# ftl/sdrainer

Measured on AMD Instinct MI355X. Metric: IQ MSamples/s through FFT+peak+envelope, higher is better.
Workload: dtype f64

## Files before the change

sdrainer_amd/csrc/bank.h:

```cpp
#pragma once
#include <hip/hip_runtime.h>

#include <algorithm>
#include <atomic>
#include <chrono>
#include <cmath>
#include <cstdio>
#include <cstdlib>
#include <cstring>
#include <memory>
#include <mutex>
#include <string>
#include <thread>
#include <vector>

#include "../../include/sdrainer_hip.h"
#include "host/delivery.h"
#include "host/frequency_mapping.h"
#include "sdr_device.h"

namespace sdrcapi {

inline thread_local std::string g_last_error;

inline int fail(int code, const std::string &msg)
{
    g_last_error = msg;
    return code;
}
#define HIP_TRY(expr)                                                                                  \
    do {                                                                                               \
        hipError_t _e = (expr);                                                                        \
        if (_e != hipSuccess)                                                                          \
            return fail(SDR_ERR_HIP, std::string(#expr) + ": " + hipGetErrorString(_e));               \
    } while (0)

template <class T>
struct DevBuf {
    T *p = nullptr;
    size_t n = 0;
    hipError_t alloc(size_t count)
    {
        n = count;
        if (count == 0)
            return hipSuccess;
        hipError_t e = hipMalloc(reinterpret_cast<void **>(&p), count * sizeof(T));
        if (e != hipSuccess)
            return e;
        e = hipMemset(p, 0, count * sizeof(T));
        if (e != hipSuccess)
            return e;
        return hipStreamSynchronize(nullptr);
    }
    void release()
    {
        if (p)
            (void)hipFree(p);
        p = nullptr;
    }
};

inline int ilog2(int n)
{
    int s = 0;
    while ((1 << s) < n)
        s++;
    return s;
}

inline const char *const kKernelNames[sdr::K_COUNT] = {"k_fft_psd",       "k_window_means", "k_noise_stats", "k_thresholds",
                                          "k_listen_gather", "k_cumulate",     "k_find_peaks",  "k_listen_decode"};

constexpr int G_THRESHOLDS = 4, N_GRAPHS = 5;
constexpr int GRAPH_PHASES = 4;
constexpr int RING = 6;
enum Stage { S_FFT = 0, S_NOISE, S_LISTEN, S_PEAKS, N_STAGES };

struct BatchSet {
    DevBuf<float> psd;
    DevBuf<float> tap;
    DevBuf<float> tapw;
    DevBuf<int32_t> tap_used;
    DevBuf<double> win_mean;
    DevBuf<sdr_frame_rec> recs;
    DevBuf<uint64_t> raw_bits, bits;
    DevBuf<sdr_edge> edges;
    DevBuf<uint32_t> edge_counts;
    DevBuf<float> tr_values;
    DevBuf<uint8_t> tr_raw, tr_deb;
    DevBuf<sdr::ListenerSlot> slots_before;
    DevBuf<float> cum_out;
    DevBuf<float> cum_part;
    DevBuf<sdr::DevPeak> dev_peaks;
    DevBuf<int> peak_counts;
    hipEvent_t done[sdr::K_COUNT] = {};
    void release()
    {
        psd.release();
        tap.release();
        tapw.release();
        tap_used.release();
        win_mean.release();
        cum_part.release();
        recs.release();
        raw_bits.release();
        bits.release();
        edges.release();
        edge_counts.release();
        tr_values.release();
        tr_raw.release();
        tr_deb.release();
        slots_before.release();
        cum_out.release();
        dev_peaks.release();
        peak_counts.release();
        for (auto &e : done) {
            if (e)
                (void)hipEventDestroy(e);
            e = nullptr;
        }
    }
};


enum Parts { PART_SPECTRA = 1, PART_LISTEN = 2, PART_ALL = 3 };

struct CursorPack {
    sdr::BatchCursor c[RING];
};

}

struct sdr_bank {
    template <class T>
    using DevBuf = sdrcapi::DevBuf<T>;
    using BatchSet = sdrcapi::BatchSet;
    static constexpr int N_STAGES = sdrcapi::N_STAGES, GRAPH_PHASES = sdrcapi::GRAPH_PHASES, N_GRAPHS = sdrcapi::N_GRAPHS, RING = sdrcapi::RING;

    sdr_config cfg{};
    int logn = 0;
    int device = 0;
    hipStream_t stream[N_STAGES] = {};
    bool own_stream[N_STAGES] = {};

    int max_chunks = 0;
    int text_cap = 2048;
    int edge_cap = 0;
    int bit_words = 0;

    DevBuf<fft64::cplx> tw;
    DevBuf<unsigned char> db_tab;
    DevBuf<int32_t> tap_bins;
    DevBuf<float> spectrum_row;
    std::vector<BatchSet> set;
    DevBuf<sdr::BandState> band_state;
    DevBuf<sdr::ListenerSlot> slots;
    DevBuf<uint16_t> morse;
    DevBuf<uint32_t> text;
    DevBuf<uint32_t> text_frames;
    DevBuf<uint32_t> edge_pos;
    DevBuf<float> carry[2];

    std::vector<sdr::BandState> h_band_state;
    std::vector<sdr::ListenerSlot> h_slots;
    std::vector<int> n_slots;
    std::vector<int64_t> center_frequency;
    int carry_cur = 0;
    int cum_count = 0;
    int64_t total_frames = 0;
    int64_t batch_index = 0;
    int last_set = 0, last_frames = 0, last_chunks = 0, last_count0 = 0;
    int last_carry_in = 0;
    int edge_width = 0;
    int find_peaks = 1;
    bool failed = false;
    DevBuf<sdr::DropCounters> drops;
    DevBuf<sdr::BatchCursor> cursors;
    hipGraph_t graph[GRAPH_PHASES][N_GRAPHS] = {};
    hipGraphExec_t graph_exec[GRAPH_PHASES][N_GRAPHS] = {};
    hipGraphNode_t graph_cursor_node[GRAPH_PHASES] = {};
    hipEvent_t phase_done[GRAPH_PHASES][N_GRAPHS] = {};
    int64_t graph_base = 0;
    int64_t graph_replays = 0;
    bool graph_ready = false;
// ... 95 lines not shown
```

sdrainer_amd/csrc/capi_bank.hip:

```cpp
#include "bank.h"
#include "twiddles.h"

using namespace sdrcapi;

namespace sdr {
int set_error(int code, const char *msg) { return fail(code, msg); }
}

namespace sdrcapi {
std::unique_ptr<host::DeliveryBackend> make_results_backend(sdr_bank *b);

void resolve_profile(sdr_bank *b)
{
    for (auto &p : b->pending) {
        float ms = 0.f;
        if (hipEventElapsedTime(&ms, p.second.first, p.second.second) == hipSuccess) {
            b->prof_ms[p.first] += ms;
            b->prof_n[p.first] += 1;
        }
        (void)hipEventDestroy(p.second.first);
        (void)hipEventDestroy(p.second.second);
    }
    b->pending.clear();
}

int sync_bank(sdr_bank *b)
{
    HIP_TRY(hipSetDevice(b->device));
    {
        const int frc = flush_late_attached(b);
        if (frc)
            return frc;
    }
    for (int s = 0; s < N_STAGES; s++)
        HIP_TRY(hipStreamSynchronize(b->stream[s]));
    resolve_profile(b);
    return SDR_OK;
}

int check_band(sdr_bank *b, int band)
{
    if (!b)
        return fail(SDR_ERR_BAD_ARG, "null bank");
    if (band < 0 || band >= b->cfg.n_bands)
        return fail(SDR_ERR_BAD_ARG, "band out of range");
    return SDR_OK;
}

int check_listener(sdr_bank *b, int band, int lid)
{
    int rc = check_band(b, band);
    if (rc)
        return rc;
    if (lid < 0 || lid >= b->n_slots[band])
        return fail(SDR_ERR_BAD_ARG, "listener id out of range");
    return SDR_OK;
}


hipError_t alloc_set(sdr_bank *b, BatchSet &S)
{
    const sdr_config &c = b->cfg;
    const size_t B = (size_t)c.n_bands, F = (size_t)c.max_batch_frames, L = (size_t)c.max_listeners, N = (size_t)c.block_size;
    hipError_t e = hipSuccess;
#define SET_ALLOC(buf, count)            \
    do {                                 \
        if (e == hipSuccess)             \
            e = (buf).alloc(count);      \
    } while (0)
    SET_ALLOC(S.psd, B * F * N);
    SET_ALLOC(S.tap, B * F * std::max<size_t>(L, 1));
    if (b->logn == 14) {
        SET_ALLOC(S.tapw, B * F * 4 * std::max<size_t>(L, 1));
        SET_ALLOC(S.tap_used, B * std::max<size_t>(L, 1));
    }
    SET_ALLOC(S.win_mean, B * F * 10);
    SET_ALLOC(S.recs, B * F);
    SET_ALLOC(S.raw_bits, B * L * (size_t)b->bit_words);
    SET_ALLOC(S.bits, B * L * (size_t)b->bit_words);
    SET_ALLOC(S.edges, B * L * (size_t)b->edge_cap);
    SET_ALLOC(S.edge_counts, B * L);
    if (c.trace) {
        SET_ALLOC(S.tr_values, B * F * L);
        SET_ALLOC(S.tr_raw, B * F * L);
        SET_ALLOC(S.tr_deb, B * F * L);
        SET_ALLOC(S.slots_before, B * L);
    }
    SET_ALLOC(S.cum_out, B * (size_t)b->max_chunks * N);
    SET_ALLOC(S.cum_part, B * (size_t)b->max_chunks * N);
    SET_ALLOC(S.dev_peaks, B * (size_t)b->max_chunks * (size_t)c.max_peaks);
    SET_ALLOC(S.peak_counts, B * (size_t)b->max_chunks);
#undef SET_ALLOC
#ifndef SDR_STAGE_EVENT_FLAGS
#define SDR_STAGE_EVENT_FLAGS hipEventDisableTiming
#endif
    for (auto &ev : S.done)
        if (e == hipSuccess)
            e = hipEventCreateWithFlags(&ev, SDR_STAGE_EVENT_FLAGS);
    return e;
}

}

extern "C" {
#pragma GCC visibility push(default)

const char *sdr_last_error(void) { return g_last_error.c_str(); }
int sdr_abi_version(void) { return SDR_ABI_VERSION; }
const char *sdr_kernel_name(int kernel) { return (kernel >= 0 && kernel < sdr::K_COUNT) ? kKernelNames[kernel] : ""; }

int sdr_self_check(int device_id)
{
    int ndev = 0;
    HIP_TRY(hipGetDeviceCount(&ndev));
    if (device_id < 0 || device_id >= ndev)
        return fail(SDR_ERR_BAD_ARG, "device_id out of range");
    int prev_dev = 0;
    HIP_TRY(hipGetDevice(&prev_dev));
    struct Restore {
        int dev;
        ~Restore() { (void)hipSetDevice(dev); }
    } restore{prev_dev};
    HIP_TRY(hipSetDevice(device_id));
    unsigned *d = nullptr, h = 0;
    HIP_TRY(hipMalloc(reinterpret_cast<void **>(&d), sizeof(unsigned)));
    hipError_t e = hipMemset(d, 0, sizeof(unsigned));
    const char *ord = getenv("SDR_SELF_CHECK_ORDER");
    if (e == hipSuccess)
        e = sdr::launch_mfma_order_probe(d, ord ? atoi(ord) : 0, nullptr);
    if (e == hipSuccess)
        e = hipMemcpy(&h, d, sizeof h, hipMemcpyDeviceToHost);
    (void)hipFree(d);
    HIP_TRY(e);
    if (h != 0)
        return fail(SDR_ERR_HIP, "self-check failed: v_mfma_f64_4x4x4 does not add its terms as a sequential, individually rounded chain on this "
                                 "device (" + std::to_string(h) + " of 4096 partial sums differ from the vector ALU's); the variance of "
                                 "FindNoiseFloor would not be bit-exact - this part is not supported");
    return SDR_OK;
}

namespace {
static int self_check_once(int device_id)
{
    constexpr int kMax = 64;
    static std::mutex mu;
    static int verdict[kMax];
    static bool done[kMax];
    static std::string message[kMax];
    if (device_id < 0 || device_id >= kMax)
        return sdr_self_check(device_id);
    std::lock_guard<std::mutex> g(mu);
    if (!done[device_id]) {
        verdict[device_id] = sdr_self_check(device_id);
        message[device_id] = g_last_error;
        done[device_id] = verdict[device_id] == SDR_OK || message[device_id].find("self-check failed") != std::string::npos;
    }
    if (verdict[device_id] != SDR_OK)
// ... 441 lines not shown
```

sdrainer_amd/csrc/capi_process.hip:

```cpp
#include <string>

#include "bank.h"

using namespace sdrcapi;

namespace sdrcapi {

constexpr int PUT_SLOTS = 16, PUT_BINS = 128;
struct SlotPack {
    int32_t n;
    int32_t index[PUT_SLOTS];
    sdr::ListenerSlot slot[PUT_SLOTS];
};
struct BinPack {
    int32_t n;
    int32_t index[PUT_BINS], bin[PUT_BINS];
};
__global__ void k_put_slots(sdr::ListenerSlot *slots, SlotPack p)
{
    constexpr int W = sizeof(sdr::ListenerSlot) / 4;
    static_assert(sizeof(sdr::ListenerSlot) % 4 == 0, "word copy");
    for (int i = threadIdx.x; i < p.n * W; i += blockDim.x)
        reinterpret_cast<uint32_t *>(slots + p.index[i / W])[i % W] = reinterpret_cast<const uint32_t *>(&p.slot[i / W])[i % W];
}
// ... 90 lines not shown
        for (int k = 0; k < sdr::K_COUNT && e[k] >= '0' && e[k] < '0' + N_STAGES; k++)
            plan[k] = e[k] - '0';
#define SDR_LAUNCH(id, call) \
    do {                     \
        if (!(diag_skip >> (id) & 1) && SDR_ON(id)) \
            HIP_TRY(call);   \
    } while (0)
#else
#define SDR_LAUNCH(id, call)  \
    do {                      \
        if (SDR_ON(id))       \
            HIP_TRY(call);    \
    } while (0)
#endif
    auto stream_of = [&](int k) { return b->stream[plan[k]]; };
    auto after = [&](int k, int dep) -> int {
        if (stream_of(k) != stream_of(dep) && !cap)
            HIP_TRY(hipStreamWaitEvent(stream_of(k), S.done[dep], 0));
        return SDR_OK;
    };
#define SDR_AFTER(k, dep)          \
    do {                           \
        int _rc = after((k), (dep)); \
        if (_rc)                   \
            return _rc;            \
    } while (0)
    static const bool stop_events = !(getenv("SDR_STOP_EVENTS") && atoi(getenv("SDR_STOP_EVENTS")) == 0);
    const bool ride = stop_events && !cap;
#define SDR_ARM(k) (sdr::t_done_event = ride ? S.done[k] : nullptr)
#define SDR_DONE(k)                                                                                   \
    do {                                                                                              \
        if ((!ride || sdr::t_done_event) && !cap) {                                                   \
            sdr::t_done_event = nullptr;                                                              \
            HIP_TRY(hipEventRecord(S.done[k], stream_of(k)));                                         \
        }                                                                                             \
    } while (0)

    static const bool host_waits = getenv("SDR_HOST_THROTTLE") && atoi(getenv("SDR_HOST_THROTTLE")) != 0;
    int max_slots = 0;
    for (int i = 0; i < B; i++)
        max_slots = std::max(max_slots, b->n_slots[i]);
    if (do_spectra) {
    static const bool park_first = !(getenv("SDR_PARK_FIRST") && atoi(getenv("SDR_PARK_FIRST")) == 0);
    if (b->results_on && !cap && park_first) {
        const int prc = b->results->park(si);
        if (prc)
            return prc;
    }
    {
        static const int launch_order[] = {sdr::K_WINDOW_MEANS, sdr::K_NOISE_STATS, sdr::K_THRESHOLDS, sdr::K_LISTEN_GATHER,
                                           sdr::K_LISTEN_DECODE, sdr::K_CUMULATE,   sdr::K_FIND_PEAKS};
        int last_on[N_STAGES];
        for (int &l : last_on)
            l = -1;
        for (int k : launch_order)
            last_on[plan[k]] = k;
        for (int st = 0; st < N_STAGES; st++) {
            const int k = last_on[st];
            if (k < 0 || st == plan[sdr::K_FFT])
                continue;
            if (cap)
                continue;
            if (hipEventQuery(S.done[k]) == hipSuccess)
                continue;
            if (host_waits)
                HIP_TRY(hipEventSynchronize(S.done[k]));
            else
                HIP_TRY(hipStreamWaitEvent(stream_of(sdr::K_FFT), S.done[k], 0));
        }
    }
    if (b->results_on && !cap && !park_first) {
        const int prc = b->results->park(si);
        if (prc)
            return prc;
    }
    if (cap && SDR_ON(sdr::K_FFT) && capture_k % RING == 0)
        HIP_TRY(launch_set_cursors(b->cursors.p + capture_k, CursorPack{}, stream_of(sdr::K_FFT)));
    {
        ProfScope ps(b, sdr::K_FFT, stream_of(sdr::K_FFT));
        SDR_ARM(sdr::K_FFT);
        sdr::FftTap tap{b->tap_bins.p, S.tap.p, max_slots, c.max_listeners};
        tap.wide = S.tapw.p;
        tap.used = S.tap_used.p;
        SDR_LAUNCH(sdr::K_FFT, sdr::launch_fft(b->logn, iq_dev, cur, b->tw.p, S.psd.p, n_frames, B, in_stride, stride, tap,
                                               stream_of(sdr::K_FFT)));
    }
    SDR_DONE(sdr::K_FFT);

    static const bool scan_path = !(getenv("SDR_NOISE_PATH") && std::string(getenv("SDR_NOISE_PATH")) == "chains");
    static const int force_exact = getenv("SDR_NOISE_FORCE_EXACT") ? atoi(getenv("SDR_NOISE_FORCE_EXACT")) : 0;
    const int scan_count0 = b->cum_count;
    int scan_slots = 1;
    if (n_frames >= SDR_CUMULATION_SIZE - scan_count0)
        scan_slots = 1 + (n_frames - (SDR_CUMULATION_SIZE - scan_count0) + SDR_CUMULATION_SIZE - 1) / SDR_CUMULATION_SIZE;
    if (cap)
        scan_slots = sdr::chunks_completed(SDR_CUMULATION_SIZE - 1, n_frames) + 1;
    const bool scan_bound = scan_path && sdr::cum_bound_pays(n_frames, B, N);
    SDR_AFTER(sdr::K_WINDOW_MEANS, sdr::K_FFT);
    {
        ProfScope ps(b, sdr::K_WINDOW_MEANS, stream_of(sdr::K_WINDOW_MEANS));
        SDR_ARM(sdr::K_WINDOW_MEANS);
        if (scan_path) {
            const sdr::CumGeom scg{N, stride, n_frames, scan_count0, b->max_chunks};
            SDR_LAUNCH(sdr::K_WINDOW_MEANS, sdr::launch_psd_scan(S.psd.p, S.recs.p, S.cum_out.p, S.cum_part.p, cur, ng, scg, scan_slots, B, scan_bound,
                                                                 force_exact, stream_of(sdr::K_WINDOW_MEANS)));
        } else {
            SDR_LAUNCH(sdr::K_WINDOW_MEANS, sdr::launch_window_means(S.psd.p, S.win_mean.p, ng, n_frames, B, stride,
                                                                     stream_of(sdr::K_WINDOW_MEANS)));
        }
    }
    SDR_DONE(sdr::K_WINDOW_MEANS);
    SDR_AFTER(sdr::K_NOISE_STATS, sdr::K_WINDOW_MEANS);
    {
        ProfScope ps(b, sdr::K_NOISE_STATS, stream_of(sdr::K_NOISE_STATS));
        SDR_ARM(sdr::K_NOISE_STATS);
        if (!scan_path)
            SDR_LAUNCH(sdr::K_NOISE_STATS, sdr::launch_noise_stats(S.psd.p, S.win_mean.p, S.recs.p, ng, n_frames, B, stride,
                                                                   stream_of(sdr::K_NOISE_STATS)));
    }
    SDR_DONE(sdr::K_NOISE_STATS);
    SDR_AFTER(sdr::K_THRESHOLDS, sdr::K_NOISE_STATS);
    {
        ProfScope ps(b, sdr::K_THRESHOLDS, stream_of(sdr::K_THRESHOLDS));
        SDR_ARM(sdr::K_THRESHOLDS);
        SDR_LAUNCH(sdr::K_THRESHOLDS, sdr::launch_thresholds(S.recs.p, b->band_state.p, n_frames, B, stride,
                                                             stream_of(sdr::K_THRESHOLDS)));
    }
    SDR_DONE(sdr::K_THRESHOLDS);
    }

    sdr::ListenGeom lg;
    lg.n = N;
    lg.stride = stride;
    lg.max_listeners = c.max_listeners;
    lg.text_cap = b->text_cap;
    lg.edge_cap = b->edge_cap;
    lg.bit_words = b->bit_words;
    lg.trace = c.trace;
    lg.frame_base = (uint32_t)first_frame;
    if (do_listen) {
    SDR_AFTER(sdr::K_LISTEN_GATHER, sdr::K_THRESHOLDS);
    SDR_AFTER(sdr::K_LISTEN_GATHER, sdr::K_FFT);
    SDR_ARM(sdr::K_LISTEN_GATHER);
    if (max_slots > 0) {
        ProfScope ps(b, sdr::K_LISTEN_GATHER, stream_of(sdr::K_LISTEN_GATHER));
        SDR_LAUNCH(sdr::K_LISTEN_GATHER, sdr::launch_listen_gather(S.tap.p, S.psd.p, S.recs.p, b->slots.p, b->db_tab.p, S.raw_bits.p, S.tr_values.p,
                                                                   S.tr_raw.p, cur, lg, n_frames, max_slots, B,
                                                                   stream_of(sdr::K_LISTEN_GATHER)));
    }
    SDR_DONE(sdr::K_LISTEN_GATHER);
    SDR_AFTER(sdr::K_LISTEN_DECODE, sdr::K_LISTEN_GATHER);
    if (c.trace && max_slots > 0 && SDR_ON(sdr::K_LISTEN_DECODE))
        HIP_TRY(hipMemcpyAsync(S.slots_before.p, b->slots.p, sizeof(sdr::ListenerSlot) * (size_t)B * (size_t)c.max_listeners,
                               hipMemcpyDeviceToDevice, stream_of(sdr::K_LISTEN_DECODE)));
    if (!b->results_on)
        SDR_ARM(sdr::K_LISTEN_DECODE);
    if (max_slots > 0) {
        ProfScope ps(b, sdr::K_LISTEN_DECODE, stream_of(sdr::K_LISTEN_DECODE));
        SDR_LAUNCH(sdr::K_LISTEN_DECODE, sdr::launch_listen_decode(b->slots.p, b->morse.p, S.raw_bits.p, S.bits.p, b->text.p,
                                                                   b->text_frames.p, S.edges.p, S.edge_counts.p, S.tr_deb.p, b->drops.p, cur,
                                                                   lg, n_frames, B, b->edge_pos.p, c.max_batch_frames, stream_of(sdr::K_LISTEN_DECODE)));
    }
    if (b->results_on && SDR_ON(sdr::K_LISTEN_DECODE)) {
        SDR_ARM(sdr::K_LISTEN_DECODE);
        HIP_TRY(sdr::launch_pack_listen(b->slots.p, S.edges.p, S.edge_counts.p, b->text.p, b->text_frames.p, b->drops.p, b->res_layout, max_slots, B,
                                        RS.block, stream_of(sdr::K_LISTEN_DECODE)));
// ... 341 lines not shown
```

sdrainer_amd/csrc/k_fft_r32.hip:

```cpp
#include <hip/hip_runtime.h>

#include <algorithm>
#include <cstdlib>
#include <mutex>

#include "fft_r32.h"
#include "sdr_device.h"

#if !defined(SDR_R32_IN_AUX)
#define SDR_R32_IN_AUX 0
#endif
#if !defined(SDR_R32_CHUNK0)
#define SDR_R32_CHUNK0 4
#endif
#if !defined(SDR_R32_PF_PLAN)
#define SDR_R32_PF_PLAN {0, 2, 2, 2, 2, 2, 2, 2, 2, 2, 2, 2, 2, 2, 2, 2, 2}
#endif
#if !defined(SDR_R32_PRIO)
#define SDR_R32_PRIO 1
#endif
#if !defined(SDR_R32_DEPTH2)
#define SDR_R32_DEPTH2 1
#endif
#if !defined(SDR_R32_CHUNK1)
#define SDR_R32_CHUNK1 2
#endif
#if !defined(SDR_R32_PRIO_FLIP2)
#define SDR_R32_PRIO_FLIP2 0
#endif
#if !defined(SDR_R32_PRIO_FLIP1)
#define SDR_R32_PRIO_FLIP1 1
#endif
#if !defined(SDR_R32_CHUNK2)
#define SDR_R32_CHUNK2 4
#endif

namespace sdr {
namespace r32 {

using fft32::cplx;
using rsrc_t = __amdgpu_buffer_rsrc_t;
typedef unsigned u32x2 __attribute__((ext_vector_type(2)));
typedef unsigned u32x4 __attribute__((ext_vector_type(4)));

__device__ __forceinline__ rsrc_t make_rsrc(const void *base, unsigned bytes)
{
    const unsigned long long b = (unsigned long long)base;
    const unsigned lo = __builtin_amdgcn_readfirstlane((unsigned)b), hi = __builtin_amdgcn_readfirstlane((unsigned)(b >> 32));
    return __builtin_amdgcn_make_buffer_rsrc((void *)(((unsigned long long)hi << 32) | lo), 0,
                                             __builtin_amdgcn_readfirstlane(bytes), 0x00020000);
}

__device__ __forceinline__ void wave_sync()
{
    __builtin_amdgcn_fence(__ATOMIC_RELEASE, "wavefront");
    __builtin_amdgcn_wave_barrier();
    __builtin_amdgcn_fence(__ATOMIC_ACQUIRE, "wavefront");
}

enum R32Stamp { RS_TOP = 0, RS_LANDED, RS_CVT, RS_FLUSHED, RS_WIDENED, RS_PASS0, RS_E0, RS_PASS1, RS_E1, RS_PASS2, RS_ROW, RS_STORED, RS_COUNT };
#if defined(SDR_R32_PHASES)
struct R32Stamps {
    unsigned v;
    bool on;
};
#define SDR_R32_STAMP(st, k)                                                                                \
    do {                                                                                                    \
        {                                                                                                   \
            const unsigned now_ = (unsigned)__builtin_amdgcn_s_memtime();                                   \
            asm volatile("v_writelane_b32 %0, %1, %2" : "+v"((st).v) : "s"(now_), "n"((int)(k)));         \
        }                                                                                                   \
    } while (0)
#else
struct R32Stamps {
};
#define SDR_R32_STAMP(st, k) \
    do {                     \
    } while (0)
#endif

constexpr int kPfPoints = 17;
constexpr int kPfPlan[kPfPoints] = SDR_R32_PF_PLAN;
constexpr int pf_begin(int point)
{
    int b = 0;
    for (int i = 0; i < point; i++)
        b += kPfPlan[i];
    return b;
}
static_assert(pf_begin(kPfPoints) == fft32::R, "the prefetch plan must cover the frame's 32 slots");
constexpr int kStorePoints = 7;
#if !defined(SDR_R32_ST_PLAN)
#define SDR_R32_ST_PLAN {2, 1, 1, 1, 1, 1, 1}
#endif
constexpr int kStPlan[kStorePoints] = SDR_R32_ST_PLAN;
constexpr int st_begin(int point)
{
    int b = 0;
    for (int i = 0; i < point; i++)
        b += kStPlan[i];
    return b;
}
static_assert(st_begin(kStorePoints) == fft32::N / 4 / fft32::T, "the store plan must cover the row's eight runs per thread");
enum PfPoint { PF_WIDENED = 0, PF_PASS0 = 1 , PF_E0 = 6 , PF_PRE1 = 10, PF_PASS1 = 11 , PF_POST2 = 15, PF_ROW = 16 };

constexpr int kTw1LdsBytes = fft32::kTw1Entries * 16;
constexpr int kSoftCounters = 4;
constexpr int kLdsBytes = fft32::kExchangeBytes + kTw1LdsBytes + kSoftCounters * 4;
enum SoftId { SOFT_ROW = 0, SOFT_E0 = 1, SOFT_E1 = 2 };
__device__ __forceinline__ void soft_arrive(unsigned *cnt)
{
    unsigned long long save;
    asm volatile("s_waitcnt lgkmcnt(0)\n\t"
                 "s_mov_b64 %0, exec\n\t"
                 "s_mov_b64 exec, 1\n\t"
                 "ds_add_u32 %1, %2\n\t"
                 "s_mov_b64 exec, %0"
                 : "=&s"(save)
                 : "v"((unsigned)(unsigned long long)cnt), "v"(1u)
                 : "memory");
}
__device__ __forceinline__ void soft_wait(unsigned *cnt, unsigned target)
{
    unsigned seen;
    asm volatile("1:\n\t"
                 "ds_read_b32 %0, %1\n\t"
                 "s_waitcnt lgkmcnt(0)\n\t"
                 "v_cmp_lt_u32_e32 vcc, %0, %2\n\t"
                 "s_cbranch_vccz 2f\n\t"
                 "s_sleep 1\n\t"
                 "s_branch 1b\n\t"
                 "2:"
                 : "=&v"(seen)
                 : "v"((unsigned)(unsigned long long)cnt), "v"(target)
                 : "vcc", "memory");
}

__device__ __forceinline__ void set_prio(int stage)
{
#if SDR_R32_PRIO
    unsigned keep;
    if (stage & 1)
        asm volatile("s_cselect_b32 %0, 1, 0\n\ts_cmp_lg_u32 m0, 0\n\ts_cbranch_scc1 1f\n\ts_setprio 1\n\ts_branch 2f\n\t1:\n\ts_setprio 0\n\t2:\n\t"
                     "s_cmp_lg_u32 %0, 0"
                     : "=&s"(keep));
    else
        asm volatile("s_cselect_b32 %0, 1, 0\n\ts_cmp_eq_u32 m0, 0\n\ts_cbranch_scc1 1f\n\ts_setprio 1\n\ts_branch 2f\n\t1:\n\ts_setprio 0\n\t2:\n\t"
                     "s_cmp_lg_u32 %0, 0"
                     : "=&s"(keep));
#endif
}

template <int E, int P>
__device__ __forceinline__ void ex_write(const double (&x)[32], int t, double *area)
{
    const int base = fft32::map_addr_thread<E, P>(t);
#pragma unroll
    for (int s = 0; s < 32; s++)
        area[base + fft32::map_addr_slot<E>(P, s)] = x[s];
}
template <int E, int P>
__device__ __forceinline__ void ex_read(double (&x)[32], int t, const double *area)
{
    const int base = fft32::map_addr_thread<E, P>(t);
#pragma unroll
    for (int s = 0; s < 32; s++)
        x[s] = area[base + fft32::map_addr_slot<E>(P, s)];
}

__global__ __launch_bounds__(fft32::T, 2) void k_fft_r32(const float *__restrict__ iq_arg, const BatchCursor *__restrict__ cur,
                                                          const cplx *__restrict__ tw, float *__restrict__ psd, int in_stride,
                                                          int out_stride, int n_frames, int fpw, const int *__restrict__ tap_bins,
                                                          float *__restrict__ tap_out, int n_tap, int tap_stride,
                                                          float *__restrict__ tap_wide, int *__restrict__ tap_used)
{
#if defined(__HIP_DEVICE_COMPILE__)
    using namespace fft32;
    extern __shared__ __attribute__((aligned(16))) unsigned char smem[];
    double *ex = reinterpret_cast<double *>(smem);
    const unsigned char *tw1_lds = smem + kExchangeBytes;
    const float *__restrict__ iq = cur ? cur->iq : iq_arg;
    const int frame0 = blockIdx.x * fpw;
    const int frame_end = min(frame0 + fpw, n_frames);
    const size_t in_band = (size_t)blockIdx.y * in_stride, out_band = (size_t)blockIdx.y * out_stride;
    const int tid = threadIdx.x;
    const rsrc_t twr = make_rsrc(tw, (unsigned)(kTwTotal * sizeof(cplx)));

    u32x2 pf[R];
    auto fetch = [&](int frame, int t, int m0, int m1) {
        const rsrc_t xrs = make_rsrc(iq + (in_band + frame) * (size_t)N * 2, frame < frame_end ? N * 8u : 0u);
        const unsigned voff = (unsigned)thread_sample(t) * 8u;
#pragma unroll
        for (int m = 0; m < R; m++)
            if (m >= m0 && m < m1)
                pf[m] = __builtin_amdgcn_raw_buffer_load_b64(xrs, voff, slot_sample(m) * 8, SDR_R32_IN_AUX);
    };
    fetch(frame0, tid, 0, R);
    for (int i = tid; i < kTw1Entries; i += T) {
        const u32x4 w = __builtin_amdgcn_raw_buffer_load_b128(twr, (unsigned)i * 16u, kTw1 * 16, 0);
        *reinterpret_cast<u32x4 *>(smem + kExchangeBytes + i * 16) = w;
    }
    const bool reg_tap = n_tap > 0 && n_tap <= T;
    const int my_bin = (reg_tap && tid < n_tap) ? tap_bins[(size_t)blockIdx.y * tap_stride + tid] : -1;
    if (tap_used && blockIdx.x == 0 && tid < tap_stride)
        tap_used[(size_t)blockIdx.y * tap_stride + tid] = my_bin;
    unsigned *soft = reinterpret_cast<unsigned *>(smem + kExchangeBytes + kTw1LdsBytes);
    if (tid < kSoftCounters)
        soft[tid] = 0;
    __syncthreads();
    R32Stamps st;
#if defined(SDR_R32_PHASES)
    st.on = false;
    st.v = 0;
#endif
    u32x4 sv[N / 4 / T];
    float tapv = 0.f;
#pragma unroll
    for (int j = 0; j < N / 4 / T; j++)
        sv[j] = u32x4{0u, 0u, 0u, 0u};
    auto flush_row = [&](int frame, int t, int j0, int j1) {
        const bool live = frame >= frame0;
        const rsrc_t pdr = make_rsrc(psd + (out_band + (live ? frame : frame0)) * (size_t)N, live ? N * 4u : 0u);
#pragma unroll
        for (int j = 0; j < N / 4 / T; j++)
            if (j >= j0 && j < j1)
                __builtin_amdgcn_raw_buffer_store_b128(sv[j], pdr, (unsigned)(t + T * j) * 16u, 0, 0);
        if (j1 == N / 4 / T) {
            const rsrc_t tpr = make_rsrc(tap_out + (out_band + (live ? frame : frame0)) * (size_t)tap_stride,
                                         (live && reg_tap) ? (unsigned)n_tap * 4u : 0u);
            __builtin_amdgcn_raw_buffer_store_b32(__float_as_uint(tapv), tpr, (unsigned)t * 4u, 0, 0);
        }
    };

#if SDR_R32_PRIO
    asm volatile("s_mov_b32 m0, %0" ::"s"(__builtin_amdgcn_readfirstlane(tid >> 8)) : "m0");
#endif
    int it = 0;
#pragma nounroll
    for (int frame = frame0; frame < frame_end; frame++, it++) {
        int t = tid;
        asm volatile("" : "+v"(t));
#if defined(SDR_R32_PHASES)
        st.on = blockIdx.x == SDR_R32_PHASES && blockIdx.y == 0 && frame == frame0 + 1;
#endif
        SDR_R32_STAMP(st, RS_TOP);
#if defined(SDR_R32_PHASES)
        asm volatile("s_waitcnt vmcnt(0)" ::: "memory");
#endif
        SDR_R32_STAMP(st, RS_LANDED);
        double xr[R], xi[R];
#pragma unroll
        for (int m = 0; m < R; m++) {
            xr[m] = (double)__uint_as_float(pf[m].x);
            xi[m] = (double)__uint_as_float(pf[m].y);
        }
#pragma unroll
        for (int m = 0; m < R; m++)
            asm volatile("" : "+v"(xr[m]), "+v"(xi[m]));
        __builtin_amdgcn_sched_barrier(0);
        auto pf_point = [&](int point) {
            __builtin_amdgcn_sched_barrier(0);
            if (point < kStorePoints)
                flush_row(frame - 1, t, st_begin(point), st_begin(point + 1));
            fetch(frame + 1, t, pf_begin(point), pf_begin(point + 1));
            __builtin_amdgcn_sched_barrier(0);
        };
#if defined(SDR_R32_PHASES)
        SDR_R32_STAMP(st, RS_CVT);
        __builtin_amdgcn_sched_barrier(0);
        flush_row(frame - 1, t, st_begin(PF_WIDENED), st_begin(PF_WIDENED + 1));
        SDR_R32_STAMP(st, RS_FLUSHED);
        fetch(frame + 1, t, pf_begin(PF_WIDENED), pf_begin(PF_WIDENED + 1));
        __builtin_amdgcn_sched_barrier(0);
#else
        pf_point(PF_WIDENED);
#endif
        SDR_R32_STAMP(st, RS_WIDENED);

        {
            const int wbase = map_addr_thread<0, 0>(t);
            run_pass<5, true, SDR_R32_CHUNK0>(
                xr, xi, [tw](int row, int) { return tw[kTw0 + row]; },
                [&](int q) {
                    set_prio(q);
                    pf_point(PF_PASS0 + q);
                    if (q == 3)
                        soft_wait(soft + SOFT_ROW, (unsigned)(NWAVES * it));
                },
                [&](int a, int b) {
                    ex[wbase + map_addr_slot<0>(0, a)] = xr[a];
                    ex[wbase + map_addr_slot<0>(0, b)] = xr[b];
                });
        }
        SDR_R32_STAMP(st, RS_PASS0);

        pf_point(PF_E0 + 0);
        __syncthreads();
        ex_read<0, 1>(xr, t, ex);
        pf_point(PF_E0 + 1);
        __syncthreads();
        ex_write<0, 0>(xi, t, ex);
        pf_point(PF_E0 + 2);
        __syncthreads();
        ex_read<0, 1>(xi, t, ex);
        pf_point(PF_E0 + 3);
        soft_arrive(soft + SOFT_E0);
        SDR_R32_STAMP(st, RS_E0);
        pf_point(PF_PRE1);

        {
            const unsigned char *row0 = tw1_lds + tw1_lo(t) * 16;
            const int wbase = map_addr_thread<1, 1>(t);
            run_pass<5, false, SDR_R32_CHUNK1>(
                xr, xi, [row0](int row, int) { return *reinterpret_cast<const cplx *>(row0 + row * 512); },
                [&](int q) {
                    set_prio(q + SDR_R32_PRIO_FLIP1);
                    if (q < 4)
                        pf_point(PF_PASS1 + q);
                    if (q == 3)
                        soft_wait(soft + SOFT_E0, (unsigned)(NWAVES * (it + 1)));
                },
                [&](int a, int b) {
                    ex[wbase + map_addr_slot<1>(1, a)] = xr[a];
                    ex[wbase + map_addr_slot<1>(1, b)] = xr[b];
                });
        }
        SDR_R32_STAMP(st, RS_PASS1);
        const unsigned tw2_off = (unsigned)tw2_pos(t, 0) * 16u;
        auto tw2 = [twr, tw2_off](int row, int u) {
            const u32x4 w = __builtin_amdgcn_raw_buffer_load_b128(twr, tw2_off, (kTw2 + row * 1024 + u * 512) * 16, 0);
            cplx r;
            r.x = __hiloint2double((int)w.y, (int)w.x);
            r.y = __hiloint2double((int)w.w, (int)w.z);
            return r;
        };
#if SDR_R32_DEPTH2 == 2
        FirstChunks2<4, SDR_R32_CHUNK2> tw2_first;
        first_chunks2<4, false, SDR_R32_CHUNK2>(tw2, tw2_first);
#else
        FirstChunk<4, SDR_R32_CHUNK2> tw2_first;
        first_chunk<4, false, SDR_R32_CHUNK2>(tw2, tw2_first);
#endif
        wave_sync();
        ex_read<1, 2>(xr, t, ex);
        wave_sync();
        ex_write<1, 1>(xi, t, ex);
        wave_sync();
        ex_read<1, 2>(xi, t, ex);
        soft_arrive(soft + SOFT_E1);
        SDR_R32_STAMP(st, RS_E1);

#if SDR_R32_DEPTH2 == 2
        run_pass2_with<4, false, SDR_R32_CHUNK2>(xr, xi, tw2_first, tw2, [&](int q) { set_prio(q + SDR_R32_PRIO_FLIP2); });
#else
        run_pass_with<4, false, SDR_R32_CHUNK2>(xr, xi, tw2_first, tw2, [&](int q) { set_prio(q + SDR_R32_PRIO_FLIP2); });
#endif
        pf_point(PF_POST2);
        SDR_R32_STAMP(st, RS_PASS2);

        {
            float p[R];
#pragma unroll
            for (int s = 0; s < R; s++)
                p[s] = (float)(xr[s] * xr[s] + xi[s] * xi[s]);
            soft_wait(soft + SOFT_E1, (unsigned)(NWAVES * (it + 1)));
            constexpr int SLOT_MASK = slot_part(2, R - 1);
            static_assert((SLOT_MASK & 0xfc) == 0, "the row swizzle reads thread bits only");
            const int tk = thread_part<2>(t) ^ ((N / 2) & ~SLOT_MASK);
            unsigned char *rowp = smem + row_word(tk) * 4;
#pragma unroll
            for (int s = 0; s < R; s++) {
                const int sk = slot_part(2, s) ^ ((N / 2) & SLOT_MASK);
                *reinterpret_cast<float *>(rowp + sk * 4) = p[s];
            }
        }
        __syncthreads();
        SDR_R32_STAMP(st, RS_ROW);
        pf_point(PF_ROW);
        {
#pragma unroll
            for (int j = 0; j < N / 4 / T; j++)
                sv[j] = *reinterpret_cast<const u32x4 *>(smem + row_word(4 * (t + T * j)) * 4);
            const float *row = reinterpret_cast<const float *>(smem);
            const float tv = row[row_word(my_bin & (N - 1))];
            tapv = my_bin >= 0 ? tv : 0.0f;
            if (__builtin_amdgcn_readfirstlane(t) < n_tap && tap_wide) {
                const rsrc_t wr = make_rsrc(tap_wide + (out_band + frame) * (size_t)(4 * tap_stride), reg_tap ? (unsigned)tap_stride * 16u : 0u);
                u32x4 wv;
                wv.x = __float_as_uint(row[row_word((my_bin - 1) & (N - 1))]);
                wv.y = __float_as_uint(tv);
                wv.z = __float_as_uint(row[row_word((my_bin + 1) & (N - 1))]);
                wv.w = 0u;
                __builtin_amdgcn_raw_buffer_store_b128(wv, wr, t < n_tap ? (unsigned)t * 16u : 0x7ffffff0u, 0, 0);
            }
        }
        soft_arrive(soft + SOFT_ROW);
        SDR_R32_STAMP(st, RS_STORED);
#if defined(SDR_R32_PHASES)
        if (st.on && (threadIdx.x & 63) < RS_COUNT)
            g_r32_phases[threadIdx.x >> 6][threadIdx.x & 63] = st.v;
#endif
    }
    flush_row(frame_end - 1, tid, 0, N / 4 / T);
#endif
}

}

static int r32_fpw(long total_frames)
{
    static const int forced = [] {
        const char *e = getenv("SDR_FFT_R32_FPW");
        return e ? std::max(1, std::min(atoi(e), 1024)) : 0;
    }();
    if (forced)
        return forced;
    return total_frames >= 4096 ? 4 : total_frames >= 2560 ? 3 : 2;
}

int r32_twiddle_count() { return fft32::kTwTotal; }
void r32_build_twiddles(const double *wre, const double *wim, fft64::cplx *out) { fft32::build_twiddles(wre, wim, out); }

hipError_t launch_fft_r32(const float *iq, const BatchCursor *cur, const fft64::cplx *tw, float *psd, int n_frames, int n_bands,
                          int in_stride, int out_stride, FftTap tap, hipStream_t stream)
{
    constexpr int kMaxDevices = 64;
    static std::once_flag attr_once[kMaxDevices];
    int dev = 0;
    hipError_t e = hipGetDevice(&dev);
    if (e != hipSuccess)
        return e;
    if (dev < 0 || dev >= kMaxDevices)
        return hipErrorInvalidDevice;
    hipError_t attr_err = hipSuccess;
    std::call_once(attr_once[dev], [&] {
        attr_err = hipFuncSetAttribute(reinterpret_cast<const void *>(&r32::k_fft_r32), hipFuncAttributeMaxDynamicSharedMemorySize,
                                       r32::kLdsBytes);
    });
    if (attr_err != hipSuccess)
        return attr_err;
    if (n_frames <= 0 || n_bands <= 0)
        return hipSuccess;
    if (tap.n > fft32::T)
        return hipErrorInvalidValue;
    int fpw = r32_fpw((long)n_frames * n_bands);
    while (fpw > 1 && (long)((n_frames + fpw - 1) / fpw) * n_bands < 256)
        fpw /= 2;
    launch_kernel(r32::k_fft_r32, dim3((n_frames + fpw - 1) / fpw, n_bands), dim3(fft32::T), r32::kLdsBytes, stream, iq, cur, tw, psd,
                  in_stride, out_stride, n_frames, fpw, tap.bins, tap.out, tap.n, tap.stride, tap.wide, tap.used);
    return hipGetLastError();
}

}
```

sdrainer_amd/csrc/sdr_device.h:

```cpp
#pragma once
#include <hip/hip_ext.h>
#include <hip/hip_runtime.h>

#include <cstdint>

#include "../../include/sdrainer_hip.h"
#include "cw_decoder.h"
#include "fft_f64.h"

namespace sdr {

struct BandState {
    float nf_ring[SDR_NOISE_WINDOW];
    float dev_ring[SDR_NOISE_WINDOW];
    float nf_sum, dev_sum;
    int32_t next;
    float peak_threshold;
};

struct ListenerSlot {
    int32_t active;
    int32_t bin;
    cw::Debouncer deb;
    cw::DecoderState dec;
// ... 1 lines not shown
    uint32_t text_dropped;
    uint32_t start_frame;
    uint32_t tapped_from;
};

struct DropCounters {
    unsigned long long runes;
    unsigned long long edges;
};

struct DevPeak {
    int32_t from, to, signal_bin;
    float signal_value;
    float y1, y2, y3;
};

struct NoiseGeom {
    int n;
    int edge;
    int window;
    int n_windows;
    double inv_n2;
};

struct BatchCursor {
    const float *iq;
    uint32_t frame_base;
    int32_t count0;
    int32_t carry_in;
    int32_t reserved;
};

struct ListenGeom {
    int n, stride, max_listeners, text_cap, edge_cap, bit_words, trace;
    uint32_t frame_base;
};

struct CumGeom {
    int n, stride, n_frames, count0, max_chunks;
};

struct ScanGeom {
    int n, edge, window, n_windows;
    int stride, n_frames, count0, max_chunks;
    int piece;
    int do_bound;
    int fpw;
    int parts;
};

struct PeakGeom {
    int n, stride, count0, max_chunks, max_peaks;
};

struct ResultsLayout {
    int max_listeners, max_chunks, max_peaks, edge_cap, text_cap;
    size_t off_peak_counts, off_peaks, off_edge_counts, off_edges, off_text_counts, off_text, off_text_frames, off_drops, bytes;
};

enum KernelId {
    K_FFT = 0, K_WINDOW_MEANS, K_NOISE_STATS, K_THRESHOLDS, K_LISTEN_GATHER, K_CUMULATE, K_FIND_PEAKS, K_LISTEN_DECODE,
    K_COUNT
};

inline thread_local hipEvent_t t_done_event = nullptr;
template <class F, class... A>
inline void launch_kernel(F kernel, dim3 grid, dim3 block, unsigned lds_bytes, hipStream_t stream, A... args)
{
    hipEvent_t done = t_done_event;
    t_done_event = nullptr;
    if (done)
        hipExtLaunchKernelGGL(kernel, grid, block, lds_bytes, stream, nullptr, done, 0, args...);
    else
        hipLaunchKernelGGL(kernel, grid, block, lds_bytes, stream, args...);
}

struct FftTap {
    const int32_t *bins;
    float *out;
    int n;
    int stride;
    float *wide = nullptr;
    int32_t *used = nullptr;
};

hipError_t launch_fft(int logn, const float *iq, const BatchCursor *cur, const fft64::cplx *tw, float *psd, int n_frames,
                      int n_bands, int in_stride, int out_stride, FftTap tap, hipStream_t stream);
int twiddle_count(int logn);
void build_twiddles(int logn, const double *wre, const double *wim, fft64::cplx *out);
hipError_t launch_fft_r32(const float *iq, const BatchCursor *cur, const fft64::cplx *tw, float *psd, int n_frames, int n_bands,
                          int in_stride, int out_stride, FftTap tap, hipStream_t stream);
int r32_twiddle_count();
void r32_build_twiddles(const double *wre, const double *wim, fft64::cplx *out);
hipError_t launch_window_means(const float *psd, double *win_mean, NoiseGeom g, int n_frames, int n_bands, int stride,
                               hipStream_t stream);
hipError_t launch_noise_stats(const float *psd, const double *win_mean, sdr_frame_rec *recs, NoiseGeom g, int n_frames,
                              int n_bands, int stride, hipStream_t stream);
hipError_t launch_mfma_order_probe(unsigned *mismatches, int order, hipStream_t stream);
hipError_t launch_thresholds(sdr_frame_rec *recs, BandState *st, int n_frames, int n_bands, int stride,
                             hipStream_t stream);
hipError_t launch_listen_gather(const float *tap, const float *psd, const sdr_frame_rec *recs, const ListenerSlot *slots, const void *db_tab,
                                uint64_t *raw_bits, float *tr_values, uint8_t *tr_raw, const BatchCursor *cur, ListenGeom g, int n_frames,
                                int n_slots, int n_bands, hipStream_t stream);
hipError_t launch_listen_decode(ListenerSlot *slots, const uint16_t *morse, const uint64_t *raw_bits,
                                uint64_t *deb_bits, uint32_t *text, uint32_t *text_frames, sdr_edge *edges,
                                uint32_t *edge_counts, uint8_t *tr_deb, DropCounters *drops, const BatchCursor *cur, ListenGeom g,
                                int n_frames, int n_bands, uint32_t *edge_pos, int pos_stride, hipStream_t stream);
hipError_t launch_listener_stop(ListenerSlot *slot, const uint16_t *morse, uint32_t *text, uint32_t *text_frames, int text_cap,
                                uint32_t frame, DropCounters *drops, hipStream_t stream);
hipError_t launch_set_debounce(ListenerSlot *slots, int n, int threshold, hipStream_t stream);
hipError_t launch_cumulate(const float *psd, const void *db_tab, float *carry0, float *carry1, int carry_in, float *cum_out,
                           const float *cum_part, const BatchCursor *cur, CumGeom g, int n_slots, int n_bands, bool bound_done, hipStream_t stream);
int scan_parts(int n_slots, int n_bands);
bool cum_bound_pays(int n_frames, int n_bands, int n);
hipError_t launch_psd_scan(const float *psd, sdr_frame_rec *recs, float *cum_out, float *cum_part, const BatchCursor *cur, NoiseGeom ng,
                           CumGeom cg, int n_slots, int n_bands, bool do_bound, int force_exact, hipStream_t stream);
hipError_t launch_noise_exact_check(const float *psd_band, sdr_frame_rec *recs_band, NoiseGeom ng, int n_frames, unsigned *mismatches,
                                    hipStream_t stream);
hipError_t launch_spectrum_row(const float *psd_row, float *out, int n, hipStream_t stream);
hipError_t launch_pack_listen(ListenerSlot *slots, const sdr_edge *edges, const uint32_t *edge_counts, const uint32_t *text,
                              const uint32_t *text_frames, const DropCounters *drops, ResultsLayout lay, int n_slots, int n_bands, unsigned char *host,
                              hipStream_t stream);
hipError_t launch_pack_peaks(const DevPeak *peaks, const int *counts, const BatchCursor *cur, ResultsLayout lay, int find_peaks,
                             int n_frames, int n_chunks, int n_bands, unsigned char *host, hipStream_t stream);
__host__ __device__ inline int chunks_completed(int count0, int n_frames)
{
    const int first_len = SDR_CUMULATION_SIZE - count0;
    return n_frames >= first_len ? 1 + (n_frames - first_len) / SDR_CUMULATION_SIZE : 0;
}
hipError_t launch_unpack_be16(const uint8_t *raw, float *out, size_t n_values, hipStream_t stream);
hipError_t launch_find_peaks(float *cum, const float *psd, const void *db_tab, const float *carry0, const float *carry1, int carry_in,
                             const sdr_frame_rec *recs, DevPeak *peaks, int *counts, const BatchCursor *cur, PeakGeom g, int n_frames,
                             int n_chunks, int n_bands, FftTap tap, hipStream_t stream);
bool fft_writes_wide_tap(int logn, int n_frames, int n_bands, int tap_n);
hipError_t launch_cumulation_row(const float *psd_band, const void *db_tab, const float *carry_in_band, float *row_out, CumGeom g, int slot,
                                 hipStream_t stream);

}
```

Measured before the change: 156,200.

## Replace static frames-per-block split in radix-32 FFT with persistent work-stealing blocks

The FFT kernel now launches roughly one block per CU per band and has each block claim frames dynamically through a per-band global atomic counter. The claim is prefetched one frame ahead and passed through LDS so the pipelined load and store overlap keeps working. The last block to finish resets the counter. This is meant to remove tail imbalance and launch overhead from the fixed frames-per-block grid. The cost is an atomic per frame, extra LDS, and a reliance on the counter being reset correctly between launches.

```diff
diff --git a/sdrainer_amd/csrc/bank.h b/sdrainer_amd/csrc/bank.h
--- a/sdrainer_amd/csrc/bank.h
+++ b/sdrainer_amd/csrc/bank.h
@@ -81,6 +81,7 @@
     DevBuf<float> tap;
     DevBuf<float> tapw;
     DevBuf<int32_t> tap_used;
+    DevBuf<uint32_t> fft_ctr;
     DevBuf<double> win_mean;
     DevBuf<sdr_frame_rec> recs;
     DevBuf<uint64_t> raw_bits, bits;
@@ -100,6 +101,7 @@
         tap.release();
         tapw.release();
         tap_used.release();
+        fft_ctr.release();
         win_mean.release();
         cum_part.release();
         recs.release();
diff --git a/sdrainer_amd/csrc/capi_bank.hip b/sdrainer_amd/csrc/capi_bank.hip
--- a/sdrainer_amd/csrc/capi_bank.hip
+++ b/sdrainer_amd/csrc/capi_bank.hip
@@ -73,6 +73,7 @@
     if (b->logn == 14) {
         SET_ALLOC(S.tapw, B * F * 4 * std::max<size_t>(L, 1));
         SET_ALLOC(S.tap_used, B * std::max<size_t>(L, 1));
+        SET_ALLOC(S.fft_ctr, B * 2);
     }
     SET_ALLOC(S.win_mean, B * F * 10);
     SET_ALLOC(S.recs, B * F);
diff --git a/sdrainer_amd/csrc/capi_process.hip b/sdrainer_amd/csrc/capi_process.hip
--- a/sdrainer_amd/csrc/capi_process.hip
+++ b/sdrainer_amd/csrc/capi_process.hip
@@ -196,6 +196,7 @@
         sdr::FftTap tap{b->tap_bins.p, S.tap.p, max_slots, c.max_listeners};
         tap.wide = S.tapw.p;
         tap.used = S.tap_used.p;
+        tap.steal = S.fft_ctr.p;
         SDR_LAUNCH(sdr::K_FFT, sdr::launch_fft(b->logn, iq_dev, cur, b->tw.p, S.psd.p, n_frames, B, in_stride, stride, tap,
                                                stream_of(sdr::K_FFT)));
     }
diff --git a/sdrainer_amd/csrc/k_fft_r32.hip b/sdrainer_amd/csrc/k_fft_r32.hip
--- a/sdrainer_amd/csrc/k_fft_r32.hip
+++ b/sdrainer_amd/csrc/k_fft_r32.hip
@@ -1,7 +1,6 @@
 #include <hip/hip_runtime.h>
 
 #include <algorithm>
-#include <cstdlib>
 #include <mutex>
 
 #include "fft_r32.h"
@@ -106,7 +105,9 @@
 
 constexpr int kTw1LdsBytes = fft32::kTw1Entries * 16;
 constexpr int kSoftCounters = 4;
-constexpr int kLdsBytes = fft32::kExchangeBytes + kTw1LdsBytes + kSoftCounters * 4;
+constexpr int kStashWords = 4;
+constexpr int kClaimBytes = fft32::T * 4;
+constexpr int kLdsBytes = fft32::kExchangeBytes + kTw1LdsBytes + (kSoftCounters + kStashWords) * 4 + kClaimBytes;
 enum SoftId { SOFT_ROW = 0, SOFT_E0 = 1, SOFT_E1 = 2 };
 __device__ __forceinline__ void soft_arrive(unsigned *cnt)
 {
@@ -168,9 +169,10 @@
         x[s] = area[base + fft32::map_addr_slot<E>(P, s)];
 }
 
+
 __global__ __launch_bounds__(fft32::T, 2) void k_fft_r32(const float *__restrict__ iq_arg, const BatchCursor *__restrict__ cur,
                                                           const cplx *__restrict__ tw, float *__restrict__ psd, int in_stride,
-                                                          int out_stride, int n_frames, int fpw, const int *__restrict__ tap_bins,
+                                                          int out_stride, int n_frames, unsigned *__restrict__ steal, const int *__restrict__ tap_bins,
                                                           float *__restrict__ tap_out, int n_tap, int tap_stride,
                                                           float *__restrict__ tap_wide, int *__restrict__ tap_used)
 {
@@ -180,22 +182,38 @@
     double *ex = reinterpret_cast<double *>(smem);
     const unsigned char *tw1_lds = smem + kExchangeBytes;
     const float *__restrict__ iq = cur ? cur->iq : iq_arg;
-    const int frame0 = blockIdx.x * fpw;
-    const int frame_end = min(frame0 + fpw, n_frames);
-    const size_t in_band = (size_t)blockIdx.y * in_stride, out_band = (size_t)blockIdx.y * out_stride;
+    const unsigned n_fr = (unsigned)n_frames;
+    constexpr unsigned kNoFrame = ~0u;
+    const size_t out_band = (size_t)blockIdx.y * out_stride;
+    const float *const iq_b = iq + (size_t)blockIdx.y * in_stride * (size_t)N * 2;
+    float *const psd_b = psd + out_band * (size_t)N, *const tap_b = tap_out + out_band * (size_t)tap_stride;
+    float *const wide_b = tap_wide ? tap_wide + out_band * (size_t)(4 * tap_stride) : nullptr;
     const int tid = threadIdx.x;
     const rsrc_t twr = make_rsrc(tw, (unsigned)(kTwTotal * sizeof(cplx)));
 
     u32x2 pf[R];
-    auto fetch = [&](int frame, int t, int m0, int m1) {
-        const rsrc_t xrs = make_rsrc(iq + (in_band + frame) * (size_t)N * 2, frame < frame_end ? N * 8u : 0u);
+    auto fetch = [&](unsigned frame, int t, int m0, int m1) {
+        const bool live = frame < n_fr;
+        const rsrc_t xrs = make_rsrc(iq_b + (size_t)frame * N * 2, live ? N * 8u : 0u);
         const unsigned voff = (unsigned)thread_sample(t) * 8u;
 #pragma unroll
         for (int m = 0; m < R; m++)
             if (m >= m0 && m < m1)
                 pf[m] = __builtin_amdgcn_raw_buffer_load_b64(xrs, voff, slot_sample(m) * 8, SDR_R32_IN_AUX);
     };
-    fetch(frame0, tid, 0, R);
+    unsigned *stash = reinterpret_cast<unsigned *>(smem + kExchangeBytes + kTw1LdsBytes + kSoftCounters * 4);
+    unsigned *claim_lds = stash + kStashWords;
+    auto band_ctr = [stash] {
+        const unsigned long long lo = (unsigned)__builtin_amdgcn_readfirstlane(stash[0]), hi = (unsigned)__builtin_amdgcn_readfirstlane(stash[1]);
+        return reinterpret_cast<unsigned *>((hi << 32) | lo);
+    };
+    if (tid == 0) {
+        unsigned *const ctr = steal + 2 * blockIdx.y;
+        stash[0] = (unsigned)(unsigned long long)ctr;
+        stash[1] = (unsigned)((unsigned long long)ctr >> 32);
+        stash[2] = gridDim.x;
+        claim_lds[0] = __hip_atomic_fetch_add(ctr, 2u, __ATOMIC_RELAXED, __HIP_MEMORY_SCOPE_AGENT);
+    }
     for (int i = tid; i < kTw1Entries; i += T) {
         const u32x4 w = __builtin_amdgcn_raw_buffer_load_b128(twr, (unsigned)i * 16u, kTw1 * 16, 0);
         *reinterpret_cast<u32x4 *>(smem + kExchangeBytes + i * 16) = w;
@@ -208,6 +226,8 @@
     if (tid < kSoftCounters)
         soft[tid] = 0;
     __syncthreads();
+    unsigned frame = __builtin_amdgcn_readfirstlane(claim_lds[0]), next = frame + 1, prev = kNoFrame;
+    fetch(frame, tid, 0, R);
     R32Stamps st;
 #if defined(SDR_R32_PHASES)
     st.on = false;
@@ -218,30 +238,34 @@
 #pragma unroll
     for (int j = 0; j < N / 4 / T; j++)
         sv[j] = u32x4{0u, 0u, 0u, 0u};
-    auto flush_row = [&](int frame, int t, int j0, int j1) {
-        const bool live = frame >= frame0;
-        const rsrc_t pdr = make_rsrc(psd + (out_band + (live ? frame : frame0)) * (size_t)N, live ? N * 4u : 0u);
+    auto flush_row = [&](unsigned frame, int t, int j0, int j1) {
+        const bool live = frame < n_fr;
+        const rsrc_t pdr = make_rsrc(psd_b + (size_t)frame * N, live ? N * 4u : 0u);
 #pragma unroll
         for (int j = 0; j < N / 4 / T; j++)
             if (j >= j0 && j < j1)
                 __builtin_amdgcn_raw_buffer_store_b128(sv[j], pdr, (unsigned)(t + T * j) * 16u, 0, 0);
         if (j1 == N / 4 / T) {
-            const rsrc_t tpr = make_rsrc(tap_out + (out_band + (live ? frame : frame0)) * (size_t)tap_stride,
+            const rsrc_t tpr = make_rsrc(tap_b + (size_t)frame * tap_stride,
                                          (live && reg_tap) ? (unsigned)n_tap * 4u : 0u);
             __builtin_amdgcn_raw_buffer_store_b32(__float_as_uint(tapv), tpr, (unsigned)t * 4u, 0, 0);
         }
     };
+    auto claim_next = [&](int t) {
+        const rsrc_t crs = make_rsrc(band_ctr(), 4u);
+        return (unsigned)__builtin_amdgcn_raw_ptr_buffer_atomic_add_i32(1, crs, (unsigned)t * 4u, 0, 0);
+    };
 
 #if SDR_R32_PRIO
     asm volatile("s_mov_b32 m0, %0" ::"s"(__builtin_amdgcn_readfirstlane(tid >> 8)) : "m0");
 #endif
     int it = 0;
 #pragma nounroll
-    for (int frame = frame0; frame < frame_end; frame++, it++) {
+    while (frame < n_fr) {
         int t = tid;
         asm volatile("" : "+v"(t));
 #if defined(SDR_R32_PHASES)
-        st.on = blockIdx.x == SDR_R32_PHASES && blockIdx.y == 0 && frame == frame0 + 1;
+        st.on = blockIdx.x == SDR_R32_PHASES && blockIdx.y == 0 && it == 1;
 #endif
         SDR_R32_STAMP(st, RS_TOP);
 #if defined(SDR_R32_PHASES)
@@ -261,20 +285,22 @@
         auto pf_point = [&](int point) {
             __builtin_amdgcn_sched_barrier(0);
             if (point < kStorePoints)
-                flush_row(frame - 1, t, st_begin(point), st_begin(point + 1));
-            fetch(frame + 1, t, pf_begin(point), pf_begin(point + 1));
+                flush_row(prev, t, st_begin(point), st_begin(point + 1));
+            fetch(next, t, pf_begin(point), pf_begin(point + 1));
             __builtin_amdgcn_sched_barrier(0);
         };
 #if defined(SDR_R32_PHASES)
         SDR_R32_STAMP(st, RS_CVT);
         __builtin_amdgcn_sched_barrier(0);
-        flush_row(frame - 1, t, st_begin(PF_WIDENED), st_begin(PF_WIDENED + 1));
+        flush_row(prev, t, st_begin(PF_WIDENED), st_begin(PF_WIDENED + 1));
         SDR_R32_STAMP(st, RS_FLUSHED);
-        fetch(frame + 1, t, pf_begin(PF_WIDENED), pf_begin(PF_WIDENED + 1));
+        fetch(next, t, pf_begin(PF_WIDENED), pf_begin(PF_WIDENED + 1));
         __builtin_amdgcn_sched_barrier(0);
 #else
         pf_point(PF_WIDENED);
 #endif
+        const unsigned claimed = claim_next(t);
+        __builtin_amdgcn_sched_barrier(0);
         SDR_R32_STAMP(st, RS_WIDENED);
 
         {
@@ -305,6 +331,7 @@
         ex_read<0, 1>(xi, t, ex);
         pf_point(PF_E0 + 3);
         soft_arrive(soft + SOFT_E0);
+        claim_lds[t] = claimed;
         SDR_R32_STAMP(st, RS_E0);
         pf_point(PF_PRE1);
 
@@ -384,8 +411,8 @@
             const float *row = reinterpret_cast<const float *>(smem);
             const float tv = row[row_word(my_bin & (N - 1))];
             tapv = my_bin >= 0 ? tv : 0.0f;
-            if (__builtin_amdgcn_readfirstlane(t) < n_tap && tap_wide) {
-                const rsrc_t wr = make_rsrc(tap_wide + (out_band + frame) * (size_t)(4 * tap_stride), reg_tap ? (unsigned)tap_stride * 16u : 0u);
+            if (__builtin_amdgcn_readfirstlane(t) < n_tap && wide_b) {
+                const rsrc_t wr = make_rsrc(wide_b + (size_t)frame * (4 * tap_stride), reg_tap ? (unsigned)tap_stride * 16u : 0u);
                 u32x4 wv;
                 wv.x = __float_as_uint(row[row_word((my_bin - 1) & (N - 1))]);
                 wv.y = __float_as_uint(tv);
@@ -394,60 +421,73 @@
                 __builtin_amdgcn_raw_buffer_store_b128(wv, wr, t < n_tap ? (unsigned)t * 16u : 0x7ffffff0u, 0, 0);
             }
         }
+        const unsigned after = __builtin_amdgcn_readfirstlane(claim_lds[0]);
         soft_arrive(soft + SOFT_ROW);
         SDR_R32_STAMP(st, RS_STORED);
 #if defined(SDR_R32_PHASES)
         if (st.on && (threadIdx.x & 63) < RS_COUNT)
             g_r32_phases[threadIdx.x >> 6][threadIdx.x & 63] = st.v;
 #endif
+        prev = frame;
+        frame = next;
+        next = after;
+        it++;
     }
-    flush_row(frame_end - 1, tid, 0, N / 4 / T);
-#endif
-}
-
-}
-
-static int r32_fpw(long total_frames)
-{
-    static const int forced = [] {
-        const char *e = getenv("SDR_FFT_R32_FPW");
-        return e ? std::max(1, std::min(atoi(e), 1024)) : 0;
-    }();
-    if (forced)
-        return forced;
-    return total_frames >= 4096 ? 4 : total_frames >= 2560 ? 3 : 2;
+    int t = tid;
+    asm volatile("" : "+v"(t));
+    flush_row(prev, t, 0, N / 4 / T);
+    if (t == 0) {
+        unsigned *const ctr = band_ctr();
+        const unsigned done = __hip_atomic_fetch_add(ctr + 1, 1u, __ATOMIC_ACQ_REL, __HIP_MEMORY_SCOPE_AGENT);
+        if (done == stash[2] - 1) {
+            __hip_atomic_store(ctr, 0u, __ATOMIC_RELAXED, __HIP_MEMORY_SCOPE_AGENT);
+            __hip_atomic_store(ctr + 1, 0u, __ATOMIC_RELAXED, __HIP_MEMORY_SCOPE_AGENT);
+        }
+    }
+#endif
+}
+
 }
 
 int r32_twiddle_count() { return fft32::kTwTotal; }
 void r32_build_twiddles(const double *wre, const double *wim, fft64::cplx *out) { fft32::build_twiddles(wre, wim, out); }
 
+#if !defined(SDR_R32_RESERVE)
+#define SDR_R32_RESERVE 0
+#endif
+
 hipError_t launch_fft_r32(const float *iq, const BatchCursor *cur, const fft64::cplx *tw, float *psd, int n_frames, int n_bands,
                           int in_stride, int out_stride, FftTap tap, hipStream_t stream)
 {
     constexpr int kMaxDevices = 64;
-    static std::once_flag attr_once[kMaxDevices];
+    static std::once_flag setup_once[kMaxDevices];
+    static hipError_t setup_err[kMaxDevices];
+    static int cu_count[kMaxDevices];
     int dev = 0;
     hipError_t e = hipGetDevice(&dev);
     if (e != hipSuccess)
         return e;
     if (dev < 0 || dev >= kMaxDevices)
         return hipErrorInvalidDevice;
-    hipError_t attr_err = hipSuccess;
-    std::call_once(attr_once[dev], [&] {
-        attr_err = hipFuncSetAttribute(reinterpret_cast<const void *>(&r32::k_fft_r32), hipFuncAttributeMaxDynamicSharedMemorySize,
-                                       r32::kLdsBytes);
+    std::call_once(setup_once[dev], [dev] {
+        hipError_t se = hipFuncSetAttribute(reinterpret_cast<const void *>(&r32::k_fft_r32), hipFuncAttributeMaxDynamicSharedMemorySize,
+                                            r32::kLdsBytes);
+        if (se == hipSuccess)
+            se = hipDeviceGetAttribute(&cu_count[dev], hipDeviceAttributeMultiprocessorCount, dev);
+        setup_err[dev] = se;
     });
-    if (attr_err != hipSuccess)
-        return attr_err;
+    if (setup_err[dev] != hipSuccess)
+        return setup_err[dev];
     if (n_frames <= 0 || n_bands <= 0)
         return hipSuccess;
     if (tap.n > fft32::T)
         return hipErrorInvalidValue;
-    int fpw = r32_fpw((long)n_frames * n_bands);
-    while (fpw > 1 && (long)((n_frames + fpw - 1) / fpw) * n_bands < 256)
-        fpw /= 2;
-    launch_kernel(r32::k_fft_r32, dim3((n_frames + fpw - 1) / fpw, n_bands), dim3(fft32::T), r32::kLdsBytes, stream, iq, cur, tw, psd,
-                  in_stride, out_stride, n_frames, fpw, tap.bins, tap.out, tap.n, tap.stride, tap.wide, tap.used);
+    if (!tap.steal)
+        return hipErrorInvalidValue;
+    const int cus = std::max(1, cu_count[dev] - SDR_R32_RESERVE);
+    const int grid = std::min((cus + n_bands - 1) / n_bands, n_frames);
+    launch_kernel(r32::k_fft_r32, dim3(grid, n_bands), dim3(fft32::T), r32::kLdsBytes, stream, iq, cur, tw, psd, in_stride, out_stride,
+                  n_frames, tap.steal, tap.bins, tap.out, tap.n, tap.stride, tap.wide, tap.used);
     return hipGetLastError();
 }
 
diff --git a/sdrainer_amd/csrc/sdr_device.h b/sdrainer_amd/csrc/sdr_device.h
--- a/sdrainer_amd/csrc/sdr_device.h
+++ b/sdrainer_amd/csrc/sdr_device.h
@@ -107,6 +107,7 @@
     int stride;
     float *wide = nullptr;
     int32_t *used = nullptr;
+    uint32_t *steal = nullptr;
 };
 
 hipError_t launch_fft(int logn, const float *iq, const BatchCursor *cur, const fft64::cplx *tw, float *psd, int n_frames,
```

Measured after the change: 169,100 (median of 6 runs). +8.3%, better.
